# aask1357/fastenhancer

Measured on AMD Instinct MI355X. Metric: audio frames/sec (hop=256, 16kHz) FastEnhancer_B, higher is better.
Workload: dtype f32

## Files before the change

fastenhancer_amd/csrc/fe_frame8.hip.h:

```cpp
#pragma once
#include "fe_kernels.hip.h"

namespace fe {

constexpr int kThreads8 = 512;
constexpr int kWaves8 = 8;

template <class S>
struct Wg8 {
    using L = Lds<S>;
    static constexpr bool MDFT = (S::NFFT == 512) || (S::C1 < 128);
    static constexpr bool OK0 = L::STAGED && L::SKIPS_LDS && S::GFLAT && S::KT == 1 && S::LOW == 0 && !S::FRNN && !S::TATT && !S::LN && !S::BIDIR &&
                               S::G8P && S::MTC == 4 && S::MT2 == 2 && MDFT && !L::PERHEAD && S::NFFT == kThreads8 && S::NTPW2 == 1;
    static constexpr int NTA = (S::NTC + 1) / 2, NTB = S::NTC - NTA;
    static constexpr int N2A = (S::NT2 + 1) / 2, N2B = S::NT2 - N2A;
    static constexpr int NPW = ceil_div(ceil_div(Pack<S>::umax(), 256), kWaves8);
    static constexpr int HPT = ceil_div(S::F2 * S::C2, kThreads8);
    static constexpr int SLOT = S::U8_SLOT;
    static constexpr int WB0 = L::NOSTAGE_TOTAL, WB1 = WB0 + 2 * SLOT;
    static constexpr int LDM = 13;
    static constexpr int MXB = L::NOSTAGE_TOTAL + 4 * SLOT, MX_FLOATS = round_up(4 * 16 * LDM + 8, 4), MXF = MXB + 4 * 16 * LDM;
    static constexpr int HST = MXB + MX_FLOATS;
    static constexpr bool HSTASH = (size_t)(HST + S::KB * S::F2 * S::C2) * 4 <= 160 * 1024;
    static constexpr size_t BYTES = (size_t)(HST + (HSTASH ? S::KB * S::F2 * S::C2 : 0)) * 4;
    static constexpr int NPWB = ceil_div(ceil_div(SLOT, 256), kWaves8);
    static constexpr bool PLAN_OK = 2 * SLOT >= Pack<S>::umax() && BYTES <= 160 * 1024 && (S::NU & 1) == 0;
    static constexpr bool OK = OK0 && PLAN_OK;
};

template <class S, int NT, int J0, int KS, int NCOLS, int LDO, bool ACT, class AF, class BF, class BI, class SIDE>
__device__ __forceinline__ void conv8(AF&& af, BF&& bf, BI&& bias, const SIDE& side, float* out, int row0, int mt, int lane, float ap = 0.0f) {
    if constexpr (NT > 0) {
        const int li = lane & 15, lg = lane >> 4;
        f32x4 acc[1][NT];
#pragma unroll
        for (int j = 0; j < NT; ++j) acc[0][j] = bias(J0 + j);
        mma_panel<1, NT, KS, Lds<S>::PDK>(acc, [&](int, int ks) { return af(ks); }, [&](int j, int ks) { return bf(J0 + j, ks); }, side);
        side.commit();
#pragma unroll
        for (int j = 0; j < NT; ++j) {
            const int col = 16 * (J0 + j) + li;
            if (col < NCOLS) {
#pragma unroll
                for (int r = 0; r < 4; ++r) {
                    const int m = 16 * mt + 4 * lg + r;
                    float v = acc[0][j][r];
                    if (ACT) v = act_scaled_f<S::EPA>(v, ap);
                    out[(row0 + m) * LDO + col] = v;
                }
            }
        }
    } else {
        constexpr int NSG = (KS + 3) / 4;
#pragma unroll
        for (int g = 0; g < NSG; ++g) side(g, NSG);
        side.commit();
    }
}
template <class S, int NA, int NB, int KS, int NCOLS, int LDO, bool ACT, class AF, class BF, class BI, class SIDE>
__device__ __forceinline__ void conv8_pair(int wh, AF&& af, BF&& bf, BI&& bias, const SIDE& side, float* out, int row0, int mt, int lane,
                                           float ap = 0.0f) {
    if (wh == 0) conv8<S, NA, 0, KS, NCOLS, LDO, ACT>(af, bf, bias, side, out, row0, mt, lane, ap);
    else conv8<S, NB, NA, KS, NCOLS, LDO, ACT>(af, bf, bias, side, out, row0, mt, lane, ap);
}

template <class S, bool DBG, bool PERSIST, bool SLOT = false, bool HIO = false, bool STRM = false>
__global__ void __launch_bounds__(kThreads8) __attribute__((amdgpu_waves_per_eu(2, 2))) fe_frame8_kernel(typename KernelArgs<SLOT, STRM>::type a_in) {
    static_assert(Wg8<S>::OK, "fe_frame8_kernel: shape outside the 512-thread kernel's plan");
    static_assert(!HIO || (SLOT && !DBG), "host audio: slotted production instantiations only");
    static_assert(!STRM || HIO, "packet audio: the host-audio instantiations only");
    typename KernelArgs<SLOT, STRM>::type a = a_in;
    if constexpr (STRM) a.T = 1;
#ifdef FE_PROBE_HOT
    if constexpr (!DBG) a.dbg = nullptr;
#else
    if constexpr (!DBG) { a.dbg = nullptr; a.clk = nullptr; }
#endif
    FE_CLK(62);
    extern __shared__ __attribute__((aligned(16))) float smem[];
    using L = Lds<S>;
    using W8 = Wg8<S>;
    constexpr int N = S::NFFT, H = S::HOP, OVL = S::OVL, F0 = S::F0, F1 = S::F1;
    constexpr int C1 = S::C1, C2 = S::C2, F2 = S::F2, HD = S::HD;
    constexpr int LDC = S::LDC, LDX = S::LDX, LDG = L::LDGX;
    constexpr int NTH = kThreads8;
#ifndef FE_WG8_PDK
#define FE_WG8_PDK 3
#endif
    constexpr int PDK = FE_WG8_PDK;

    const int tid0 = threadIdx.x;
    const int tid = tid0;
    const int lane = tid & 63;
    const int wave0 = __builtin_amdgcn_readfirstlane(tid >> 6);
    const int wave = wave0;
    float hv = 0.0f;
    auto hop_issue = [&](int bb) {
        if constexpr (STRM) {
            const StreamView v = stream_view<H>(a, bb);
            if (v.hops && tid0 >= OVL) hv = stream_sample(a.wav_in, a.format, v.in_off + (tid0 - OVL));
        } else
        if constexpr (HIO) { if (bb < a.B && tid0 >= OVL) hv = a.wav_in[(size_t)bb * a.in_stride + tid0 - OVL]; }
    };
    hop_issue((int)blockIdx.x);
    const float* __restrict__ wp = a.wp;
    WSrc<true> wb;
    constexpr PackedOffsets o = Pack<S>::v;
    wb.rsrc = __builtin_amdgcn_make_buffer_rsrc(const_cast<float*>(a.wp), 0, o.total * 4, 0x00020000);
    wb.lane4 = lane * 4;
    wb.li4 = (lane & 15) * 4;
    wb.lds = nullptr;
    wb.base = 0;
    wb.k4d = 0;
    float ap = 0.0f;
    if constexpr (S::EPP) ap = wp[o.act_p];

    float* sc = smem + L::SC;
    float* Ebuf = smem + L::E;
    float* W0 = smem + L::W0;
    float* W1 = smem + L::W1;
    float2* tw = reinterpret_cast<float2*>(smem + L::TW);
    constexpr int NPW = W8::NPW;
    DmaJobT<NPW> job;
    job.l = smem + W8::WB0;
    job.rsrc = wb.rsrc;
    job.soff = (o.u_off[0] + wave * 256) * 4;
    job.wave = wave;
    job.lane = lane;
    typename Dft<S>::FwdConst dc;
    float fv = 0.0f, fw = 0.0f;
    {
        const StageSide<NPW, o.u_size[0] / 256, kWaves8> st0{&job};
        st0(0, 1);
        float2 twv = make_float2(0.0f, 0.0f);
        if (tid < N / 2) twv = reinterpret_cast<const float2*>(wp + o.twiddle)[tid];
        DmaJobT<NPW> job1 = job;
        job1.l = smem + W8::WB1;
        job1.soff = (o.u_off[1] + wave * 256) * 4;
        const StageSide<NPW, PERSIST ? 0 : o.u_size[1] / 256, kWaves8> st1{&job1};
        if constexpr (!PERSIST) {
            const int b0 = (int)blockIdx.x;
            if constexpr (SLOT) {
                int s0;
                bool live;
                if constexpr (STRM) {
                    const StreamView v0 = stream_view<H>(a, b0);
                    s0 = v0.slot;
                    live = v0.hops != 0 && (unsigned)s0 < (unsigned)a.capacity;
                } else {
                    s0 = a.slots[b0];
                    live = (unsigned)s0 < (unsigned)a.capacity;
                }
                if constexpr (HIO) fv = (tid < OVL) ? (live ? a.cache_stft[(size_t)s0 * OVL + tid] : 0.0f) : hv;
                else fv = (tid < OVL) ? (live ? a.cache_stft[(size_t)s0 * OVL + tid] : 0.0f) : a.wav_in[(size_t)b0 * a.in_stride + tid - OVL];
            } else {
                fv = (tid < OVL) ? a.cache_stft[(size_t)b0 * OVL + tid] : a.wav_in[(size_t)b0 * a.in_stride + tid - OVL];
            }
            fw = wp[o.window + tid];
            if (wave < 4) Dft<S>::load(dc, wb, o, wave);
            st1(0, 1);
        }
        for (int i = tid; i < 2 * S::LDS_S; i += NTH) smem[L::SC + i] = 0.0f;
        for (int i = tid; i < (S::NL + 1) * 2 * LDC; i += NTH) {
            const int e = i / (2 * LDC), q = i - e * (2 * LDC);
            smem[L::E + e * S::ACT + (q >= LDC ? (F1 + 1) * LDC + (q - LDC) : q)] = 0.0f;
        }
        if (tid < N / 2) tw[tid] = twv;
        if (tid < 8) smem[W8::MXF + tid] = 0.0f;
        st0.commit();
        if constexpr (!PERSIST) {
            st1.commit();
            smem[L::FFT_A + tid] = fv * fw;
        }
    }
    __syncthreads();

    int b = (int)blockIdx.x;
    int fc = 0;
    StreamView sv{-1, 0, 0, 0};
#pragma unroll 1
    do {
        int sb = b;
        int nst = a.B;
        if constexpr (SLOT) {
            static_assert(!DBG, "slotted step: production instantiations only");
            if constexpr (STRM) {
                sv = stream_view<H>(a, b);
                sb = sv.slot;
            } else
            sb = a.slots[b];
            nst = a.capacity;
            if constexpr (STRM) {
                if (sv.hops == 0 || (unsigned)sb >= (unsigned)nst) {
                    if (sv.hops) stream_zero_row(a.wav_out, a.format, sv.out_off, H, tid0, NTH);
                    __builtin_amdgcn_s_waitcnt(0);
                    b += (int)gridDim.x;
                    hop_issue(b);
                    continue;
                }
            } else
            if ((unsigned)sb >= (unsigned)nst) {
                if constexpr (HIO) { if (tid0 < H) __builtin_nontemporal_store(0.0f, a.wav_out + (size_t)b * a.out_stride + tid0); }
                else
                if (tid0 < H) a.wav_out[(size_t)b * a.out_stride + tid0] = 0.0f;
                __builtin_amdgcn_s_waitcnt(0);
                b += (int)gridDim.x;
                hop_issue(b);
                continue;
            }
        }
        int lz = 0, lzv = 0;
        if constexpr (PERSIST) { asm volatile("" : "+s"(lz)); asm volatile("" : "+v"(lzv)); }
        const int wave = wave0 + lz;
        const int tid = tid0 + lzv;
        const int lane = tid & 63;
        const int ws = wave & 3, wh = wave >> 2;
        const int li = lane & 15, lg = lane >> 4;
        float* cst = a.cache_stft + (size_t)sb * OVL;
        float* cis = a.cache_istft + (size_t)sb * OVL;
        const int fpar = (S::NU & 1) ? (fc & 1) : 0;
#define FE8_BEGIN_UNIT(U)                                                                          \
        constexpr int fe_un_ = ((U) + 1 == S::NU) ? 0 : (U) + 1;                                   \
        {                                                                                          \
            const int slot_ = ((U) & 1) ^ fpar;                                                    \
            job.l = smem + (slot_ ? W8::WB0 : W8::WB1);                                            \
            job.soff = (o.u_off[fe_un_] + wave * 256) * 4;                                         \
            wb.lds = smem + (slot_ ? W8::WB1 : W8::WB0);                                           \
            wb.base = o.u_off[(U)];                                                                \
        }                                                                                          \
        const StageSide<NPW, ((!PERSIST && ((U) + 1 == S::NU || (U) == 0)) || (U) == S::U_RFPRE + 1) ? 0 : o.u_size[fe_un_] / 256, kWaves8> stage{&job}
        FE_CLK(0);
        float* q0 = smem + L::FFT_A;
        float* q1 = q0 + N;
        float* q3 = smem + L::FFT_B + N;
        {
            if constexpr (PERSIST) {
                if (wave < 4) Dft<S>::load(dc, wb, o, wave);
                const float* xin = a.wav_in + (size_t)b * a.in_stride;
                if constexpr (HIO) {
                    fv = (tid < OVL) ? cst[tid] : hv;
                    hop_issue(b + (int)gridDim.x);
                } else
                fv = (tid < OVL) ? cst[tid] : xin[tid - OVL];
                fw = wp[o.window + tid];
                q0[tid] = fv * fw;
                __syncthreads();
            }
            if (tid >= H) cst[tid - H] = fv;
            FE_CLK(1);
            float* nyq = a.dbg ? a.dbg + (size_t)b * a.dbg_stride + DebugLayout<S>::offset(0) + 2 * F0 : nullptr;
            if (wave < 4) Dft<S>::template forward<false>(q0, q3, tw, dc, wave, lane, nyq);
            __syncthreads();
            FE_CLK(2);
            const float* Xr = q3;
            const float* Xi = q3 + N / 2;
            if (a.dbg) {
                float* dst = a.dbg + (size_t)b * a.dbg_stride + DebugLayout<S>::offset(0);
                for (int f = tid; f < F0; f += NTH) { dst[2 * f] = Xr[f]; dst[2 * f + 1] = Xi[f]; }
            }
            for (int f = tid; f < F0; f += NTH) {
                const float re = Xr[f], im = Xi[f];
                const float mag = fmaxf(sqrtf(re * re + im * im), 1.0e-5f);
                const float g = pow_f(mag, a.compression - 1.0f);
                sc[2 + f] = re * g;
                sc[S::LDS_S + 2 + f] = im * g;
            }
        }
        __syncthreads();
        if (a.dbg) {
            float* dst = a.dbg + (size_t)b * a.dbg_stride + DebugLayout<S>::offset(1);
            for (int f = tid; f < F0; f += NTH) { dst[2 * f] = sc[2 + f]; dst[2 * f + 1] = sc[S::LDS_S + 2 + f]; }
        }

        FE_CLK(3);
        {
            FE8_BEGIN_UNIT(0);
            conv8_pair<S, W8::NTA, W8::NTB, 4, C1, LDC, true>(
                wh,
                [&](int ks) {
                    const int kk = 4 * ks + lg;
                    const int c = kk & 1, s = (kk >> 1) & 3, tp = kk >> 3;
                    return sc[c * S::LDS_S + 4 * (16 * ws + li + tp) + s];
                },
                [&](int j, int ks) { return wb.at(o.enc_pre_w + (j * 4 + ks) * 64); },
                [&](int j) { return wb.at16x4(o.enc_pre_b + j * 64); }, stage, Ebuf, 1, ws, lane, ap);
        }
        __syncthreads();
        dbg_dump<S, NTH>(a, b, 2, Ebuf + LDC, LDC);

        FE_CLK(4);
        static_for<S::NL>([&](auto l_) {
            constexpr int l = decltype(l_)::value;
            const float* in = Ebuf + l * S::ACT;
            float* out = Ebuf + (l + 1) * S::ACT;
            if (l == 0) FE_CLK(40);
            {
                FE8_BEGIN_UNIT(S::U_ENC + l);
                const float* const t0 = in + (16 * ws + li) * LDC + lg;
                conv8_pair<S, W8::NTA, W8::NTB, 3 * S::KS_C, C1, LDC, true>(
                    wh, [&](int ks) { return t0[(ks / S::KS_C) * LDC + 4 * (ks % S::KS_C)]; },
                    [&](int j, int ks) { return wb.at(o.enc_w[l] + (j * (3 * S::KS_C) + ks) * 64); },
                    [&](int j) { return wb.at16x4(o.enc_b[l] + j * 64); }, stage, out, 1, ws, lane, ap);
            }
            if (l == 0) FE_CLK(42);
            __syncthreads();
            if (l == 0) FE_CLK(43);
            dbg_dump<S, NTH>(a, b, 3 + l, out + LDC, LDC);
        });

        float* Xb = smem + L::X;
        float* Hl = smem + L::HL;
        float* Hs = smem + L::HS;
        float* Gi = smem + L::GI;
        float* Y1 = smem + L::Y1;
        float* Y2 = smem + L::Y2;

        FE_CLK(5);
        constexpr int NTPW3 = S::NTPW3;
        constexpr int HPT = W8::HPT;
        constexpr int K2 = S::KS_2;
        f32x4 xr;
        const int g_rt = wave & 1;
        const int g_t0 = wave < 4 ? 3 * (wave >> 1) : 3 * S::G8_NG;
        const float* const sGx = smem + W8::WB0 + 1 * W8::SLOT;
        const float* const sGh = smem + W8::WB0 + 3 * W8::SLOT;
        const float* const sF = smem + W8::WB0 + 0 * W8::SLOT;
        const float* const sQ = smem + W8::WB0 + 2 * W8::SLOT;
        constexpr int NPWB = W8::NPWB;
        DmaJobT<NPWB> jb1, jb2;
        jb1.rsrc = wb.rsrc; jb1.wave = wave; jb1.lane = lane; jb1.l = smem; jb1.soff = 0;
        jb2 = jb1;
        auto stage_to = [&](DmaJobT<NPWB>& j, int src_floats, int dst_floats) { j.l = smem + dst_floats; j.soff = (src_floats + wave * 256) * 4; };
        constexpr int u8_stride = S::KB > 1 ? o.u8_gx[1] - o.u8_gx[0] : 0;
        using StG = StageSide<NPWB, S::U8_G / 256, kWaves8>;
        using StF = StageSide<NPWB, S::U8_F / 256, kWaves8>;
        using StQ = StageSide<NPWB, S::U8_Q / 256, kWaves8>;
        float pe_r[4];
        auto tok_dst = [&](float* base) {
            const int col = 16 * ws + li;
            return base + (16 * wh + 4 * lg) * LDX + (col < C2 ? col : C2);
        };
        int hs_off[HPT];
#pragma unroll
        for (int q = 0; q < HPT; ++q) {
            const int i = tid + q * NTH, f = i / C2;
            hs_off[q] = i < F2 * C2 ? f * LDX + (i - f * C2) : C2;
        }
        {
            constexpr int KS = F1 / 4;
            const float* Ein = Ebuf + S::NL * S::ACT + LDC;
            FE8_BEGIN_UNIT(S::U_RFPRE);
            stage_to(jb1, o.u8_gx[0], W8::WB0 + 1 * W8::SLOT);
            const StG stg{&jb1};
            f32x4 acc[1][1];
            acc_init_zero<1, 1>(acc);
            const int nt = ws < S::NTC ? ws : S::NTC - 1;
            mma_panel<1, 1, KS, PDK>(
                acc, [&](int, int ks) { return wb.at(o.rfpre_lin + (wh * KS + ks) * 64); },
                [&](int, int ks) { return Ein[(4 * ks + lg) * LDC + 16 * nt + li]; }, side2(stage, stg));
            stage.commit();
            stg.commit();
            const int col = 16 * ws + li;
            if (ws < S::NTC && col < C1 && 16 * wh + 4 * lg < F2) {
#pragma unroll
                for (int r = 0; r < 4; ++r) Y1[(16 * wh + 4 * lg + r) * LDC + col] = acc[0][0][r];
            }
        }
        __syncthreads();
        {
            FE8_BEGIN_UNIT(S::U_RFPRE + 1);
            stage_to(jb1, o.u8_gh[0], W8::WB0 + 3 * W8::SLOT);
            const StG stg{&jb1};
            float hpre[HPT];
            const float* hg0 = a.h + (size_t)sb * (F2 * C2);
#pragma unroll
            for (int q = 0; q < HPT; ++q) { const int i = tid + q * NTH; hpre[q] = hg0[i < F2 * C2 ? i : F2 * C2 - 1]; }
            f32x4 acc[1][1];
            const int nt = ws < S::NT2 ? ws : S::NT2 - 1;
            acc[0][0] = wb.at16x4(o.rfpre_b + nt * 64);
            const float* ya = Y1 + (16 * wh + li) * LDC + lg;
            mma_panel<1, 1, S::KS_C, PDK>(
                acc, [&](int, int ks) { return ya[4 * ks]; },
                [&](int, int ks) { return wb.at(o.rfpre_w + (nt * S::KS_C + ks) * 64); }, stg);
            (void)stage;
            stg.commit();
            xr = acc[0][0];
            float* xd = tok_dst(Xb);
#pragma unroll
            for (int r = 0; r < 4; ++r) xd[r * LDX] = acc[0][0][r];
#pragma unroll
            for (int q = 0; q < HPT; ++q) Hs[hs_off[q]] = hpre[q];
        }
        __syncthreads();
        dbg_dump<S, NTH>(a, b, 3 + S::NL, Xb, LDX);

        FE_CLK(6);
#pragma unroll
        for (int k = 0; k < S::KB; ++k) {
            float* hg = a.h + ((size_t)k * nst + sb) * (F2 * C2);
            const int ub = k * u8_stride;
            if (k == 0) FE_CLK(20);
            {
                stage_to(jb1, o.u8_f1[0] + ub, W8::WB0 + 0 * W8::SLOT);
                stage_to(jb2, o.u8_q[0] + ub, W8::WB0 + 2 * W8::SLOT);
                const StF st1{&jb1};
                const StQ st2{&jb2};
                const auto sideg = side2(st1, st2);
                if (k == 0) {
#pragma unroll
                    for (int r = 0; r < 4; ++r) {
                        const int row = 16 * wh + 4 * lg + r, col = 16 * ws + li;
                        pe_r[r] = wb.gather_g(o.blk_pe + (row < F2 ? row : F2 - 1) * C2 + (col < C2 ? col : C2 - 1));
                    }
                }
                const float* xa = Xb + (16 * g_rt + li) * LDX + lg;
                const float* ha = Hs + (16 * g_rt + li) * LDX + lg;
                const float* wx = sGx + g_t0 * (K2 * 64) + lane;
                const float* wh_ = sGh + g_t0 * (K2 * 64) + lane;
                const float* bx = sGx + S::G8_NT * K2 * 64 + g_t0 * 16 + li;
                const float* bh = sGh + S::G8_NT * K2 * 64 + g_t0 * 16 + li;
                __builtin_amdgcn_sched_barrier(0);
                if (k == 0) FE_CLK(45);
                if (wave < 4) {
                    const int ch = 16 * (wave >> 1) + li;
                    float hprev[4];
#pragma unroll
                    for (int r = 0; r < 4; ++r) hprev[r] = Hs[(16 * g_rt + 4 * lg + r) * LDX + ch];
                    const float b0 = bx[0], b1 = bx[16], b2 = bx[32], b3 = bh[32];
                    f32x4 ar = f32x4{b0, b0, b0, b0}, az = f32x4{b1, b1, b1, b1};
                    f32x4 anx = f32x4{b2, b2, b2, b2}, anh = f32x4{b3, b3, b3, b3};
                    mma_panel_sel<1, 3, 2 * K2, PDK>(
                        [&](int, int j, int ks) -> f32x4& { return j == 0 ? ar : (j == 1 ? az : (ks < K2 ? anx : anh)); },
                        [&](int, int ks) { return ks < K2 ? xa[4 * ks] : ha[4 * (ks - K2)]; },
                        [&](int j, int ks) { return ks < K2 ? wx[(j * K2 + ks) * 64] : wh_[(j * K2 + (ks - K2)) * 64]; }, sideg);
                    __builtin_amdgcn_sched_barrier(0);
                    if (k == 0) FE_CLK(46);
                    float hn[4];
#pragma unroll
                    for (int r = 0; r < 4; ++r) {
                        const float rr = sigmoid_pre(ar[r]);
                        const float zz = sigmoid_pre(az[r]);
                        const float nn = tanh_pre(__builtin_fmaf(rr, anh[r], anx[r]));
                        hn[r] = __builtin_fmaf(zz, hprev[r] - nn, nn);
                    }
                    if (16 * g_rt + 4 * lg < F2) {
#pragma unroll
                        for (int r = 0; r < 4; ++r) {
                            const int row = 16 * g_rt + 4 * lg + r;
                            Hl[row * LDX + ch] = hn[r];
                            if constexpr (W8::HSTASH) smem[W8::HST + k * (F2 * C2) + row * C2 + ch] = hn[r];
                            else hg[row * C2 + ch] = hn[r];
                        }
                    }
                } else {
                    constexpr int R = S::G8_R, LDM = W8::LDM;
                    const bool hhalf = wave >= 6;
                    float* mx = smem + W8::MXB + ((hhalf ? 2 : 0) + g_rt) * (16 * LDM);
                    int* mflag = reinterpret_cast<int*>(smem + W8::MXF) + g_rt;
                    const int seq = fc * S::KB + k + 1;
                    f32x4 s0, s1 = f32x4{0.0f, 0.0f, 0.0f, 0.0f};
                    __builtin_amdgcn_s_setprio(3);
                    if (!hhalf) {
                        const float b0 = bx[0];
                        s0 = f32x4{b0, b0, b0, b0};
                        mma_panel_sel<1, 1, K2, PDK>([&](int, int, int ks) -> f32x4& { return (ks & 1) ? s1 : s0; },
                                                     [&](int, int ks) { return xa[4 * ks]; }, [&](int, int ks) { return wx[ks * 64]; }, sideg);
                    } else {
                        const float b1 = bh[0];
                        s0 = f32x4{b1, b1, b1, b1};
                        mma_panel_sel<1, 1, K2, PDK>([&](int, int, int ks) -> f32x4& { return ((ks + K2) & 1) ? s1 : s0; },
                                                     [&](int, int ks) { return ha[4 * ks]; }, [&](int, int ks) { return wh_[ks * 64]; }, sideg);
                    }
                    s0 += s1;
                    __builtin_amdgcn_sched_barrier(0);
                    if (k == 0) FE_CLK(46);
                    if (li < 3 * R) {
#pragma unroll
                        for (int r = 0; r < 4; ++r) mx[(4 * lg + r) * LDM + li] = s0[r];
                    }
                    if (!hhalf) {
                        __atomic_signal_fence(__ATOMIC_SEQ_CST);
                        __builtin_amdgcn_s_waitcnt(0xc07f);
                        if (lane == 0) __hip_atomic_store(mflag, seq, __ATOMIC_RELAXED, __HIP_MEMORY_SCOPE_WORKGROUP);
                        __atomic_signal_fence(__ATOMIC_SEQ_CST);
                    } else {
                        const int row = lane >> 2, c = lane & 3;
                        static_assert(R == 4, "one (row, channel) per lane: sixteen rows x four channels");
                        const int ch = 16 * S::G8_NG + c;
                        const bool live = 16 * g_rt + row < F2;
                        const float hprev = Hs[(16 * g_rt + row) * LDX + ch];
                        __atomic_signal_fence(__ATOMIC_SEQ_CST);
                        while (__builtin_amdgcn_readfirstlane(__hip_atomic_load(mflag, __ATOMIC_RELAXED, __HIP_MEMORY_SCOPE_WORKGROUP)) < seq) {}
                        __atomic_signal_fence(__ATOMIC_SEQ_CST);
                        const float* mxx = smem + W8::MXB + g_rt * (16 * LDM) + row * LDM + c;
                        const float* mxh = mx + row * LDM + c;
                        const float sxr = mxx[0], sxz = mxx[R], sxn = mxx[2 * R];
                        const float shr = mxh[0], shz = mxh[R], shn = mxh[2 * R];
                        const float rr = sigmoid_pre(sxr + shr);
                        const float zz = sigmoid_pre(sxz + shz);
                        const float nn = tanh_pre(__builtin_fmaf(rr, shn, sxn));
                        const float hn = __builtin_fmaf(zz, hprev - nn, nn);
                        if (live) {
                            Hl[(16 * g_rt + row) * LDX + ch] = hn;
                            if constexpr (W8::HSTASH) smem[W8::HST + k * (F2 * C2) + (16 * g_rt + row) * C2 + ch] = hn;
                            else hg[(16 * g_rt + row) * C2 + ch] = hn;
                        }
                    }
                    __builtin_amdgcn_s_setprio(0);
                }
                st1.commit();
                st2.commit();
            }
            if (k == 0) FE_CLK(47);
            __syncthreads();
            if (k == 0) FE_CLK(21);
            if (k == 0) FE_CLK(22);
            const int ntf = ws < S::NT2 ? ws : S::NT2 - 1;
            {
                stage_to(jb1, o.u8_gx[0] + ub + u8_stride, W8::WB0 + 1 * W8::SLOT);
                const StG stn{&jb1};
                f32x4 acc[1][1];
                const float bj = sF[S::NT2 * K2 * 64 + ntf * 16 + li];
                acc[0][0] = f32x4{bj, bj, bj, bj};
                const float* hla = Hl + (16 * wh + li) * LDX + lg;
                const float* wf = sF + ntf * (K2 * 64) + lane;
                if (k + 1 < S::KB) {
                    mma_panel<1, 1, K2, PDK>(acc, [&](int, int ks) { return hla[4 * ks]; }, [&](int, int ks) { return wf[ks * 64]; }, stn);
                    stn.commit();
                } else
                    mma_panel<1, 1, K2, PDK>(acc, [&](int, int ks) { return hla[4 * ks]; }, [&](int, int ks) { return wf[ks * 64]; }, NoSide{});
                float* xd = tok_dst(Xb);
#pragma unroll
                for (int r = 0; r < 4; ++r) {
                    float v = acc[0][0][r] + xr[r];
                    if (k == 0) v += pe_r[r];
                    xr[r] = v;
                    xd[r * LDX] = v;
                }
            }
            __syncthreads();
            dbg_dump<S, NTH>(a, b, 4 + S::NL + 2 * k, Xb, LDX);
            if (k == 0) FE_CLK(23);
            {
                stage_to(jb1, o.u8_f2[0] + ub, W8::WB0 + 0 * W8::SLOT);
                const StF st1{&jb1};
                f32x4 acc[1][NTPW3];
                acc_init_zero<1, NTPW3>(acc);
                __builtin_amdgcn_sched_barrier(0);
                if (k == 0) FE_CLK(50);
                const float* xa = Xb + (16 * wh + li) * LDX + lg;
                mma_panel<1, NTPW3, K2, PDK>(acc, [&](int, int ks) { return xa[4 * ks]; },
                                             [&](int j, int ks) {
                                                 int nt = ws + 4 * j;
                                                 nt = nt < S::NT3 ? nt : S::NT3 - 1;
                                                 return sQ[(nt * K2 + ks) * 64 + lane];
                                             }, st1);
                st1.commit();
                __builtin_amdgcn_sched_barrier(0);
                if (k == 0) FE_CLK(51);
                float* gdst = Gi + (16 * wh + 4 * lg) * LDG + 16 * ws + li;
#pragma unroll
                for (int j = 0; j < NTPW3; ++j)
                    if (ws + 4 * j < S::NT3) {
#pragma unroll
                        for (int r = 0; r < 4; ++r) gdst[r * LDG + 64 * j] = acc[0][j][r];
                    }
                __builtin_amdgcn_sched_barrier(0);
                if (k == 0) FE_CLK(52);
            }
            __syncthreads();
            if (k == 0) FE_CLK(24);
            attention_head<S, 1, LDG>(Gi, Hl, ws * 3 * HD, ws, wh, 1, lane);
            __syncthreads();
            if (k == 0) FE_CLK(25);
            {
                float hpre[HPT];
                if (k + 1 < S::KB) {
                    const float* hgn = hg + (size_t)nst * (F2 * C2);
#pragma unroll
                    for (int q = 0; q < HPT; ++q) { const int i = tid + q * NTH; hpre[q] = hgn[i < F2 * C2 ? i : F2 * C2 - 1]; }
                }
                f32x4 acc[1][1];
                const float bj = sF[S::NT2 * K2 * 64 + ntf * 16 + li];
                acc[0][0] = f32x4{bj, bj, bj, bj};
                const float* hla = Hl + (16 * wh + li) * LDX + lg;
                const float* wf = sF + ntf * (K2 * 64) + lane;
                if (k + 1 < S::KB) {
                    stage_to(jb1, o.u8_gh[0] + ub + u8_stride, W8::WB0 + 3 * W8::SLOT);
                    const StG stn{&jb1};
                    mma_panel<1, 1, K2, PDK>(acc, [&](int, int ks) { return hla[4 * ks]; }, [&](int, int ks) { return wf[ks * 64]; }, stn);
                    stn.commit();
                } else {
                    stage_to(jb1, o.u_off[S::U_RFPOST], W8::WB1);
                    const StageSide<NPWB, o.u_size[S::U_RFPOST] / 256, kWaves8> stn{&jb1};
                    mma_panel<1, 1, K2, PDK>(acc, [&](int, int ks) { return hla[4 * ks]; }, [&](int, int ks) { return wf[ks * 64]; }, stn);
                    stn.commit();
                }
                if (k + 1 < S::KB) {
#pragma unroll
                    for (int q = 0; q < HPT; ++q) Hs[hs_off[q]] = hpre[q];
                }
                float* xd = tok_dst(Xb);
#pragma unroll
                for (int r = 0; r < 4; ++r) {
                    const float v = acc[0][0][r] + xr[r];
                    xr[r] = v;
                    xd[r * LDX] = v;
                }
            }
            __syncthreads();
            if (k == 0) FE_CLK(26);
            dbg_dump<S, NTH>(a, b, 5 + S::NL + 2 * k, Xb, LDX);
        }

        FE_CLK(7);
        {
            constexpr int KS = F2 / 4;
            FE8_BEGIN_UNIT(S::U_RFPOST);
            conv8_pair<S, W8::N2A, W8::N2B, KS, C2, LDX, false>(
                wh, [&](int ks) { return wb.at(o.rfpost_lin + (ws * KS + ks) * 64); },
                [&](int j, int ks) { return Xb[(4 * ks + lg) * LDX + 16 * j + li]; },
                [&](int) { return f32x4{0.0f, 0.0f, 0.0f, 0.0f}; }, stage, Y2, 0, ws, lane);
        }
        __syncthreads();
        float* const Wx = W1;
        float* const Wy = W0;
        for (int i = tid; i < 2 * LDC; i += NTH) {
            const int r = i / LDC, c = i - r * LDC;
            Wy[(r ? F1 + 1 : 0) * LDC + c] = 0.0f;
        }
        if (a.dbg != nullptr) {
            float* dst = a.dbg + (size_t)b * a.dbg_stride + DebugLayout<S>::offset(4 + S::NL + 2 * S::KB);
            for (int i = tid; i < F1 * C1; i += NTH) {
                const int f = i / C1, n = i - f * C1;
                float v = wp[o.rfpost_b + n];
                for (int kk = 0; kk < C2; ++kk) v += Y2[f * LDX + kk] * wp[o.rfpost_w + n * C2 + kk];
                dst[i] = v;
            }
        }

        FE_CLK(8);
        static_for<S::NL>([&](auto l_) {
            constexpr int l = decltype(l_)::value;
            const float* skip = Ebuf + (S::NL - l) * S::ACT;
            {
                FE8_BEGIN_UNIT(S::U_DEC + l * 2);
                constexpr bool FOLD0 = (l == 0);
                constexpr int K0 = FOLD0 ? S::KS_2 : S::KS_C;
                const float* xa = FOLD0 ? Y2 + (16 * ws + li) * LDX + lg : Wx + (16 * ws + li + 1) * LDC + lg;
                const float* sk = skip + (16 * ws + li + 1) * LDC + lg;
                conv8_pair<S, W8::NTA, W8::NTB, K0 + S::KS_C, C1, LDC, true>(
                    wh, [&](int ks) { return ks < K0 ? xa[4 * ks] : sk[4 * (ks - K0)]; },
                    [&](int j, int ks) { return wb.at(o.dec1_w[l] + (j * (K0 + S::KS_C) + ks) * 64); },
                    [&](int j) { return wb.at16x4(o.dec1_b[l] + j * 64); }, stage, Wy, 1, ws, lane, ap);
            }
            __syncthreads();
            {
                FE8_BEGIN_UNIT(S::U_DEC + l * 2 + 1);
                const float* const t0 = Wy + (16 * ws + li) * LDC + lg;
                conv8_pair<S, W8::NTA, W8::NTB, 3 * S::KS_C, C1, LDC, true>(
                    wh, [&](int ks) { return t0[(ks / S::KS_C) * LDC + 4 * (ks % S::KS_C)]; },
                    [&](int j, int ks) { return wb.at(o.dec3_w[l] + (j * (3 * S::KS_C) + ks) * 64); },
                    [&](int j) { return wb.at16x4(o.dec3_b[l] + j * 64); }, stage, Wx, 1, ws, lane, ap);
            }
            __syncthreads();
            dbg_dump<S, NTH>(a, b, 5 + S::NL + 2 * S::KB + l, Wx + LDC, LDC);
        });

        FE_CLK(9);
        float* PT = smem + L::PT;
        typename Dft<S>::InvConst idc;
        float mb0 = 0.0f, mb1 = 0.0f;
        {
            FE8_BEGIN_UNIT(S::U_POST);
            const float* xa = Wx + (16 * ws + li + 1) * LDC + lg;
            const float* sk = Ebuf + (16 * ws + li + 1) * LDC + lg;
            conv8_pair<S, W8::NTA, W8::NTB, 2 * S::KS_C, C1, LDC, true>(
                wh, [&](int ks) { return ks < S::KS_C ? xa[4 * ks] : sk[4 * (ks - S::KS_C)]; },
                [&](int j, int ks) { return wb.at(o.post1_w + (j * (2 * S::KS_C) + ks) * 64); },
                [&](int j) { return wb.at16x4(o.post1_b + j * 64); }, stage, Wy, 1, ws, lane, ap);
        }
        __syncthreads();
        {
            FE8_BEGIN_UNIT(S::U_POST + 1);
            const float* xa = Wy + (16 * ws + li + 1) * LDC + lg;
            conv8_pair<S, 1, 0, S::KS_C, 16, S::LDP, false>(
                wh, [&](int ks) { return xa[4 * ks]; }, [&](int j, int ks) { return wb.at(o.post_t_w + (j * S::KS_C + ks) * 64); },
                [&](int) { return f32x4{0.0f, 0.0f, 0.0f, 0.0f}; }, stage, PT, 0, ws, lane);
            if (wave < 4) Dft<S>::load(idc, wb, o, wave);
            mb0 = wb.scalar(o.post_t_b);
            mb1 = wb.scalar(o.post_t_b + 1);
        }
        __syncthreads();

        FE_CLK(10);
        {
            const float b0 = mb0, b1 = mb1;
            for (int f = tid; f < F0; f += NTH) {
                const int q = f + 2, j1 = q & 3, i1 = q >> 2;
                float m0 = b0, m1 = b1;
                if (i1 < F1) { m0 += PT[i1 * S::LDP + j1]; m1 += PT[i1 * S::LDP + 8 + j1]; }
                if (i1 >= 1) { m0 += PT[(i1 - 1) * S::LDP + j1 + 4]; m1 += PT[(i1 - 1) * S::LDP + 8 + j1 + 4]; }
                if constexpr (S::EPM != kMaskNone) { m0 = mask_f<S::EPM>(m0); m1 = mask_f<S::EPM>(m1); }
                const float xr_ = sc[2 + f], xi_ = sc[S::LDS_S + 2 + f];
                float yr = xr_ * m0 - xi_ * m1;
                float yi = xr_ * m1 + xi_ * m0;
                if (a.dbg) {
                    float* dst = a.dbg + (size_t)b * a.dbg_stride + DebugLayout<S>::offset(5 + 2 * S::NL + 2 * S::KB);
                    dst[2 * f] = m0; dst[2 * f + 1] = m1;
                }
                const float mag = sqrtf(yr * yr + yi * yi);
                const float g = pow_f(mag, 1.0f / a.compression - 1.0f);
                yr *= g; yi *= g;
                if (a.dbg) {
                    float* dst = a.dbg + (size_t)b * a.dbg_stride + DebugLayout<S>::offset(6 + 2 * S::NL + 2 * S::KB);
                    dst[2 * f] = yr; dst[2 * f + 1] = yi;
                    if (f == 0) { dst[2 * F0] = 0.0f; dst[2 * F0 + 1] = 0.0f; }
                }
                q3[f] = yr;
                q3[N / 2 + f] = yi;
            }
        }
        __syncthreads();

        FE_CLK(11);
        {
            const float ow = wp[o.window_istft + tid];
            const float oc = tid < OVL ? cis[tid] : 0.0f;
            if (wave < 4) Dft<S>::template inverse<WSrc<true>, false>(q3, q0, q1, tw, idc, wb, o, wave, lane);
            __syncthreads();
            FE_CLK(12);
            const int pi = Dft<S>::pidx(tid & (Dft<S>::N1 - 1), tid / Dft<S>::N1);
            const float xo = (q0[pi] + q1[pi]) * ow + oc;
            if constexpr (STRM) {
                if (a.format) {
                    const int qv = pcm16_out(xo);
                    const int pw = pcm16_pair(qv, __shfl_down(qv, 1));
                    const int p1 = __shfl_down(pw, 2), p2 = __shfl_down(pw, 4), p3 = __shfl_down(pw, 6);
                    short* orow = reinterpret_cast<short*>(a.wav_out) + sv.out_off;
                    if (tid < H) {
                        if (H % 8 == 0 && (reinterpret_cast<size_t>(orow) & 15) == 0) {
                            if ((tid & 7) == 0) __builtin_nontemporal_store(i32x4{pw, p1, p2, p3}, reinterpret_cast<i32x4*>(orow + tid));
                        } else {
                            __builtin_nontemporal_store((short)qv, orow + tid);
                        }
                    }
                } else {
                    const float x1 = __shfl_down(xo, 1), x2 = __shfl_down(xo, 2), x3 = __shfl_down(xo, 3);
                    float* orow = a.wav_out + sv.out_off;
                    if (tid < H) {
                        if (H % 4 == 0 && (reinterpret_cast<size_t>(orow) & 15) == 0) {
                            if ((tid & 3) == 0) __builtin_nontemporal_store(f32x4{xo, x1, x2, x3}, reinterpret_cast<f32x4*>(orow + tid));
                        } else {
                            __builtin_nontemporal_store(xo, orow + tid);
                        }
                    }
                }
                if (tid >= H) cis[tid - H] = xo;
            } else
            if constexpr (HIO) {
                const float x1 = __shfl_down(xo, 1), x2 = __shfl_down(xo, 2), x3 = __shfl_down(xo, 3);
                float* orow = a.wav_out + (size_t)b * a.out_stride;
                if (tid < H) {
                    if (H % 4 == 0 && (reinterpret_cast<size_t>(orow) & 15) == 0) {
                        if ((tid & 3) == 0) __builtin_nontemporal_store(f32x4{xo, x1, x2, x3}, reinterpret_cast<f32x4*>(orow + tid));
                    } else {
                        __builtin_nontemporal_store(xo, orow + tid);
                    }
                }
                else cis[tid - H] = xo;
            } else {
            if (tid < H) a.wav_out[(size_t)b * a.out_stride + tid] = xo;
            else cis[tid - H] = xo;
            }
            if constexpr (W8::HSTASH) {
                constexpr int N4 = F2 * C2 / 4;
                static_assert((F2 * C2) % 4 == 0 && W8::HST % 4 == 0, "16-byte state rows");
                const f32x4* hst = reinterpret_cast<const f32x4*>(smem + W8::HST);
#pragma unroll
                for (int k = 0; k < S::KB; ++k) {
                    f32x4* dst = reinterpret_cast<f32x4*>(a.h + ((size_t)k * nst + sb) * (F2 * C2));
                    for (int e = tid; e < N4; e += NTH) dst[e] = hst[k * N4 + e];
                }
            }
            if constexpr (PERSIST) __syncthreads();
        }
        FE_CLK(13);
        b += (int)gridDim.x;
        ++fc;
    } while (PERSIST && b < a.B);
#undef FE8_BEGIN_UNIT
    FE_CLK(63);
}

}
```

Measured before the change: 8.304 million.

## Precompute decoder skip-connection partial products inside attention heads

Moves the skip-input half of each decoder/post conv (whose input Ebuf is already known) into the RoFormer block loop, interleaving those MFMAs with the attention softmax stages via a new attention_head_fill routine using setprio/sched_barrier. The partial results are carried in registers (ska) and used as bias for the later convs, which then only process the non-skip K range. This aims to fill latency gaps in attention and shorten the decoder; it costs extra register pressure in a 2-waves-per-EU kernel and extra LDS staging of weight pieces.

```diff
diff --git a/fastenhancer_amd/csrc/fe_frame8.hip.h b/fastenhancer_amd/csrc/fe_frame8.hip.h
--- a/fastenhancer_amd/csrc/fe_frame8.hip.h
+++ b/fastenhancer_amd/csrc/fe_frame8.hip.h
@@ -25,6 +25,11 @@
     static constexpr size_t BYTES = (size_t)(HST + (HSTASH ? S::KB * S::F2 * S::C2 : 0)) * 4;
     static constexpr int NPWB = ceil_div(ceil_div(SLOT, 256), kWaves8);
     static constexpr bool PLAN_OK = 2 * SLOT >= Pack<S>::umax() && BYTES <= 160 * 1024 && (S::NU & 1) == 0;
+    static constexpr int SK_PIECES = S::NTC * S::KS_C / 4, SK_PT = S::KS_C / 4;
+    static constexpr int SK_NPI = ceil_div(SK_PIECES, kWaves8);
+    static constexpr int SKB = WB0 + S::U8_F;
+    static constexpr bool SKIPF = S::KS_C % 4 == 0 && S::U8_F + SK_PIECES * 256 <= SLOT;
+    static constexpr int NSKP = !SKIPF ? 0 : (S::NL + 1 < S::KB ? S::NL + 1 : S::KB);
     static constexpr bool OK = OK0 && PLAN_OK;
 };
 
@@ -62,6 +67,138 @@
                                            float ap = 0.0f) {
     if (wh == 0) conv8<S, NA, 0, KS, NCOLS, LDO, ACT>(af, bf, bias, side, out, row0, mt, lane, ap);
     else conv8<S, NB, NA, KS, NCOLS, LDO, ACT>(af, bf, bias, side, out, row0, mt, lane, ap);
+}
+
+template <class S, int LDG, int NT, int KSF>
+__device__ __forceinline__ void attention_head_fill(const float* G, float* Hl, int hoff, int head, int qt, int lane, f32x4* facc, const float* fa,
+                                                    const float* fb) {
+    constexpr int HD = S::HD, F2 = S::F2, LDX = S::LDX, MT2 = S::MT2;
+    constexpr int KSD = ceil_div(HD, 4);
+    constexpr int MTD = ceil_div(HD, 16);
+    constexpr int KC = ceil_div(KSF, 3);
+    const int li = lane & 15, lg = lane >> 4;
+    float xa[2][KC], xb[2][NT > 0 ? NT : 1][KC];
+    auto fload = [&](auto c_) {
+        constexpr int c = decltype(c_)::value;
+#pragma unroll
+        for (int kk = 0; kk < KC; ++kk) {
+            const int ks = c * KC + kk;
+            if (NT > 0 && ks < KSF) {
+                xa[c & 1][kk] = fa[4 * ks];
+#pragma unroll
+                for (int j = 0; j < NT; ++j) xb[c & 1][j][kk] = fb[(j * KSF + ks) * 64];
+            }
+        }
+    };
+    auto fmma = [&](auto c_) {
+        constexpr int c = decltype(c_)::value;
+#pragma unroll
+        for (int kk = 0; kk < KC; ++kk)
+            if (c * KC + kk < KSF) {
+#pragma unroll
+                for (int j = 0; j < NT; ++j) facc[j] = FE_MFMA(xa[c & 1][kk], xb[c & 1][j][kk], facc[j]);
+            }
+    };
+    using I0 = std::integral_constant<int, 0>;
+    using I1 = std::integral_constant<int, 1>;
+    using I2 = std::integral_constant<int, 2>;
+    __builtin_amdgcn_sched_barrier(0);
+    __builtin_amdgcn_s_setprio(3);
+    float ka[MT2][KSD], qb[KSD];
+#pragma unroll
+    for (int ks = 0; ks < KSD; ++ks) {
+#pragma unroll
+        for (int i = 0; i < MT2; ++i) ka[i][ks] = G[(16 * i + li) * LDG + hoff + HD + 4 * ks + lg];
+        const int d = 4 * ks + lg;
+        const float v = G[(16 * qt + li) * LDG + hoff + (d < HD ? d : HD - 1)];
+        qb[ks] = d < HD ? v : 0.0f;
+    }
+    __builtin_amdgcn_sched_barrier(0);
+    __builtin_amdgcn_s_setprio(0);
+    fload(I0{});
+    __builtin_amdgcn_sched_barrier(0);
+    __builtin_amdgcn_s_setprio(3);
+    f32x4 sacc[MT2];
+#pragma unroll
+    for (int i = 0; i < MT2; ++i) sacc[i] = f32x4{0.0f, 0.0f, 0.0f, 0.0f};
+#pragma unroll
+    for (int ks = 0; ks < KSD; ++ks)
+#pragma unroll
+        for (int i = 0; i < MT2; ++i) sacc[i] = FE_MFMA(ka[i][ks], qb[ks], sacc[i]);
+    float av[MT2][4][MTD];
+#pragma unroll
+    for (int i = 0; i < MT2; ++i)
+#pragma unroll
+        for (int r = 0; r < 4; ++r) {
+            int key = 16 * i + 4 * lg + r;
+            key = key < F2 ? key : F2 - 1;
+#pragma unroll
+            for (int md = 0; md < MTD; ++md) {
+                int d = 16 * md + li;
+                d = d < HD ? d : HD - 1;
+                av[i][r][md] = G[key * LDG + hoff + 2 * HD + d];
+            }
+        }
+    __builtin_amdgcn_sched_barrier(0);
+    __builtin_amdgcn_s_setprio(0);
+    fmma(I0{});
+    fload(I1{});
+    __builtin_amdgcn_sched_barrier(0);
+    __builtin_amdgcn_s_setprio(3);
+    const float scale = rsqrtf((float)HD) * 1.4426950408889634f;
+    float mx = -INFINITY;
+#pragma unroll
+    for (int i = 0; i < MT2; ++i)
+#pragma unroll
+        for (int r = 0; r < 4; ++r) {
+            const int key = 16 * i + 4 * lg + r;
+            float sv = sacc[i][r];
+            if (16 * i + 15 >= F2) sv = key < F2 ? sv : -INFINITY;
+            sacc[i][r] = sv;
+            mx = fmaxf(mx, sv);
+        }
+    mx = rows_allreduce(mx, [](float p, float q) { return fmaxf(p, q); }) * scale;
+    __builtin_amdgcn_sched_barrier(0);
+    __builtin_amdgcn_s_setprio(0);
+    fmma(I1{});
+    fload(I2{});
+    __builtin_amdgcn_sched_barrier(0);
+    __builtin_amdgcn_s_setprio(3);
+    float sum = 0.0f;
+#pragma unroll
+    for (int i = 0; i < MT2; ++i)
+#pragma unroll
+        for (int r = 0; r < 4; ++r) {
+            const float p = __builtin_amdgcn_exp2f(__builtin_fmaf(sacc[i][r], scale, -mx));
+            sacc[i][r] = p;
+            sum += p;
+        }
+    sum = rows_allreduce(sum, [](float p, float q) { return p + q; });
+    const float inv_sum = __builtin_amdgcn_rcpf(sum);
+    __builtin_amdgcn_sched_barrier(0);
+    __builtin_amdgcn_s_setprio(0);
+    fmma(I2{});
+    __builtin_amdgcn_sched_barrier(0);
+    __builtin_amdgcn_s_setprio(3);
+    f32x4 oacc[MTD];
+#pragma unroll
+    for (int md = 0; md < MTD; ++md) oacc[md] = f32x4{0.0f, 0.0f, 0.0f, 0.0f};
+#pragma unroll
+    for (int i = 0; i < MT2; ++i)
+#pragma unroll
+        for (int r = 0; r < 4; ++r)
+#pragma unroll
+            for (int md = 0; md < MTD; ++md) oacc[md] = FE_MFMA(av[i][r][md], sacc[i][r], oacc[md]);
+    const int q = 16 * qt + li;
+#pragma unroll
+    for (int md = 0; md < MTD; ++md)
+#pragma unroll
+        for (int r = 0; r < 4; ++r) {
+            const int d = 16 * md + 4 * lg + r;
+            if (d < HD && q < F2) Hl[q * LDX + head * HD + d] = oacc[md][r] * inv_sum;
+        }
+    __builtin_amdgcn_s_setprio(0);
+    __builtin_amdgcn_sched_barrier(0);
 }
 
 template <class S, bool DBG, bool PERSIST, bool SLOT = false, bool HIO = false, bool STRM = false>
@@ -216,6 +353,7 @@
         const int lane = tid & 63;
         const int ws = wave & 3, wh = wave >> 2;
         const int li = lane & 15, lg = lane >> 4;
+        if constexpr (PERSIST) { wb.lane4 = lane * 4; wb.li4 = li * 4; }
         float* cst = a.cache_stft + (size_t)sb * OVL;
         float* cis = a.cache_istft + (size_t)sb * OVL;
         const int fpar = (S::NU & 1) ? (fc & 1) : 0;
@@ -395,6 +533,9 @@
         dbg_dump<S, NTH>(a, b, 3 + S::NL, Xb, LDX);
 
         FE_CLK(6);
+        constexpr int NSKP = W8::NSKP;
+        f32x4 ska[NSKP > 0 ? NSKP : 1][W8::NTA];
+        float* const skw = smem + W8::SKB;
 #pragma unroll
         for (int k = 0; k < S::KB; ++k) {
             float* hg = a.h + ((size_t)k * nst + sb) * (F2 * C2);
@@ -546,6 +687,24 @@
                 const StF st1{&jb1};
                 f32x4 acc[1][NTPW3];
                 acc_init_zero<1, NTPW3>(acc);
+                f32x4 skr[W8::SK_NPI];
+                static_for<NSKP>([&](auto p_) {
+                    constexpr int p = decltype(p_)::value;
+                    if (p == k) {
+                        constexpr int K0 = p == 0 ? S::KS_2 : S::KS_C;
+                        constexpr int wofs = (p < S::NL ? o.dec1_w[p < S::NL ? p : 0] : o.post1_w) + K0 * 64, bofs = p < S::NL ? o.dec1_b[p < S::NL ? p : 0] : o.post1_b;
+#pragma unroll
+                        for (int i = 0; i < W8::SK_NPI; ++i) {
+                            const int pc = wave + kWaves8 * i, j = pc / W8::SK_PT, q = pc - j * W8::SK_PT;
+                            skr[i] = wb.at_gv4(wofs + j * ((K0 + S::KS_C) * 64) + q * 256, pc < W8::SK_PIECES ? lane * 16 : 0x40000000);
+                        }
+#pragma unroll
+                        for (int j = 0; j < W8::NTA; ++j) {
+                            const int nt = (wh ? W8::NTA : 0) + j;
+                            ska[p][j] = wb.at_gv4(bofs + (nt < S::NTC ? nt : S::NTC - 1) * 64, wb.li4 * 4);
+                        }
+                    }
+                });
                 __builtin_amdgcn_sched_barrier(0);
                 if (k == 0) FE_CLK(50);
                 const float* xa = Xb + (16 * wh + li) * LDX + lg;
@@ -556,6 +715,13 @@
                                                  return sQ[(nt * K2 + ks) * 64 + lane];
                                              }, st1);
                 st1.commit();
+                if (k < NSKP) {
+#pragma unroll
+                    for (int i = 0; i < W8::SK_NPI; ++i) {
+                        const int pc = wave + kWaves8 * i;
+                        if (pc < W8::SK_PIECES) *reinterpret_cast<f32x4*>(skw + pc * 256 + lane * 4) = skr[i];
+                    }
+                }
                 __builtin_amdgcn_sched_barrier(0);
                 if (k == 0) FE_CLK(51);
                 float* gdst = Gi + (16 * wh + 4 * lg) * LDG + 16 * ws + li;
@@ -570,7 +736,17 @@
             }
             __syncthreads();
             if (k == 0) FE_CLK(24);
-            attention_head<S, 1, LDG>(Gi, Hl, ws * 3 * HD, ws, wh, 1, lane);
+            if (k < NSKP) {
+                static_for<NSKP>([&](auto p_) {
+                    constexpr int p = decltype(p_)::value;
+                    if (p == k) {
+                        const float* ska_ = Ebuf + (S::NL - p) * S::ACT + (16 * ws + li + 1) * LDC + lg;
+                        if (wh == 0) attention_head_fill<S, LDG, W8::NTA, S::KS_C>(Gi, Hl, ws * 3 * HD, ws, 0, lane, ska[p], ska_, skw + lane);
+                        else attention_head_fill<S, LDG, W8::NTB, S::KS_C>(Gi, Hl, ws * 3 * HD, ws, 1, lane, ska[p], ska_, skw + W8::NTA * S::KS_C * 64 + lane);
+                    }
+                });
+            } else
+                attention_head<S, 1, LDG>(Gi, Hl, ws * 3 * HD, ws, wh, 1, lane);
             __syncthreads();
             if (k == 0) FE_CLK(25);
             {
@@ -649,6 +825,12 @@
                 constexpr int K0 = FOLD0 ? S::KS_2 : S::KS_C;
                 const float* xa = FOLD0 ? Y2 + (16 * ws + li) * LDX + lg : Wx + (16 * ws + li + 1) * LDC + lg;
                 const float* sk = skip + (16 * ws + li + 1) * LDC + lg;
+                if constexpr (l < NSKP) {
+                    auto af = [&](int ks) { return xa[4 * ks]; };
+                    auto bf = [&](int j, int ks) { return wb.at(o.dec1_w[l] + (j * (K0 + S::KS_C) + ks) * 64); };
+                    if (wh == 0) conv8<S, W8::NTA, 0, K0, C1, LDC, true>(af, bf, [&](int j) { return ska[l][j]; }, stage, Wy, 1, ws, lane, ap);
+                    else conv8<S, W8::NTB, W8::NTA, K0, C1, LDC, true>(af, bf, [&](int j) { return ska[l][j - W8::NTA]; }, stage, Wy, 1, ws, lane, ap);
+                } else
                 conv8_pair<S, W8::NTA, W8::NTB, K0 + S::KS_C, C1, LDC, true>(
                     wh, [&](int ks) { return ks < K0 ? xa[4 * ks] : sk[4 * (ks - K0)]; },
                     [&](int j, int ks) { return wb.at(o.dec1_w[l] + (j * (K0 + S::KS_C) + ks) * 64); },
@@ -675,6 +857,13 @@
             FE8_BEGIN_UNIT(S::U_POST);
             const float* xa = Wx + (16 * ws + li + 1) * LDC + lg;
             const float* sk = Ebuf + (16 * ws + li + 1) * LDC + lg;
+            if constexpr (S::NL < NSKP) {
+                auto af = [&](int ks) { return xa[4 * ks]; };
+                auto bf = [&](int j, int ks) { return wb.at(o.post1_w + (j * (2 * S::KS_C) + ks) * 64); };
+                constexpr int pp = S::NL < NSKP ? S::NL : 0;
+                if (wh == 0) conv8<S, W8::NTA, 0, S::KS_C, C1, LDC, true>(af, bf, [&](int j) { return ska[pp][j]; }, stage, Wy, 1, ws, lane, ap);
+                else conv8<S, W8::NTB, W8::NTA, S::KS_C, C1, LDC, true>(af, bf, [&](int j) { return ska[pp][j - W8::NTA]; }, stage, Wy, 1, ws, lane, ap);
+            } else
             conv8_pair<S, W8::NTA, W8::NTB, 2 * S::KS_C, C1, LDC, true>(
                 wh, [&](int ks) { return ks < S::KS_C ? xa[4 * ks] : sk[4 * (ks - S::KS_C)]; },
                 [&](int j, int ks) { return wb.at(o.post1_w + (j * (2 * S::KS_C) + ks) * 64); },
```

Result: slower. 8.151 million (-1.8%).
